# thygate/stable-diffusion-webui-depthmap-script

Hardware: NVIDIA H100
Metric: images/sec (higher is better)
Workload: dtype fp16

## Files before the change

### stable-diffusion-webui-depthmap-script_b200/csrc/attention_wgmma.cu

```cuda
#include <cuda.h>
#include <cuda_fp16.h>
#include <math.h>

#include "common.cuh"
#include "tc_common.cuh"

namespace dm {
using namespace tc;

__device__ __forceinline__ float ex2_approx(float x) {
    float y;
    asm("ex2.approx.ftz.f32 %0, %1;" : "=f"(y) : "f"(x));
    return y;
}

int make_tmap_2d(CUtensorMap *tm, const void *ptr, uint64_t rows, uint64_t cols, uint64_t ld, uint32_t box_rows, uint32_t box_cols);

struct AttnParams {
    int B, N, H;
    int C;
    float scale_log2e;
    const __half *bias;
    int bias_ld;
    __half *out;
    const float *rel_table;
    int nrd, gh, gw;
    int sub_stride;
};

constexpr int AT_BQ = 128, AT_BKV = 128, AT_D = 64, AT_STAGES = 2;
constexpr int AT_THREADS = 384;
constexpr int AT_Q_BYTES = AT_BQ * AT_D * 2;
constexpr int AT_KV_BYTES = AT_BKV * AT_D * 2;
constexpr int AT_K_OFF = AT_Q_BYTES;
constexpr int AT_V_OFF = AT_K_OFF + AT_STAGES * AT_KV_BYTES;
constexpr int AT_BAR_OFF = AT_V_OFF + AT_STAGES * AT_KV_BYTES;
constexpr int AT_TAB_OFF = AT_BAR_OFF + 64;
constexpr int AT_SMEM_MAX = 227 * 1024;
constexpr int AT_STAGERS = 96;

static inline int relpos_sub_stride(int gh, int gw) {
    const int span = gh < (AT_BQ - 1) / gw + 2 ? gh : (AT_BQ - 1) / gw + 2;
    return ((2 * span - 1) * (2 * gw - 1) + 1 + 3) & ~3;
}

template <int BIAS_MODE>
__global__ void __launch_bounds__(AT_THREADS, 1) attention_wgmma_kernel(const __grid_constant__ CUtensorMap tmQKV, AttnParams p) {
    extern __shared__ __align__(1024) uint8_t smem_raw[];
    uint8_t *sQ = smem_raw, *sK = smem_raw + AT_K_OFF, *sV = smem_raw + AT_V_OFF;
    uint64_t *bars = reinterpret_cast<uint64_t *>(smem_raw + AT_BAR_OFF);
    uint64_t *q_full = bars, *kv_full = bars + 1, *kv_empty = bars + 1 + AT_STAGES;
    float *s_tab = reinterpret_cast<float *>(smem_raw + AT_TAB_OFF);
    int *s_koff = reinterpret_cast<int *>(s_tab + AT_STAGES * p.sub_stride);

    const int warp = threadIdx.x >> 5, lane = threadIdx.x & 31;
    const int q0 = blockIdx.x * AT_BQ, h = blockIdx.y, b = blockIdx.z;
    const int num_kv = (p.N + AT_BKV - 1) / AT_BKV;
    const int row_base = b * p.N;

    if (threadIdx.x == 0) {
        prefetch_tmap(&tmQKV);
        mbar_init(q_full, 1);
        for (int s = 0; s < AT_STAGES; ++s) {
            mbar_init(&kv_full[s], BIAS_MODE == 2 ? 1 + AT_STAGERS : 1);
            mbar_init(&kv_empty[s], 8);
        }
        fence_barrier_init();
    }
    __syncthreads();

    if (warp < 4) {
        if (threadIdx.x == 0) {
            mbar_arrive_expect_tx(q_full, AT_Q_BYTES);
            tma_load_2d(sQ, &tmQKV, q_full, h * AT_D, row_base + q0);
            for (int j = 0; j < num_kv; ++j) {
                const int s = j % AT_STAGES;
                mbar_wait(&kv_empty[s], ((j / AT_STAGES) & 1) ^ 1);
                mbar_arrive_expect_tx(&kv_full[s], 2 * AT_KV_BYTES);
                tma_load_2d(sK + s * AT_KV_BYTES, &tmQKV, &kv_full[s], p.C + h * AT_D, row_base + j * AT_BKV);
                tma_load_2d(sV + s * AT_KV_BYTES, &tmQKV, &kv_full[s], 2 * p.C + h * AT_D, row_base + j * AT_BKV);
            }
        } else if (BIAS_MODE == 2 && warp >= 1) {
            const int st = threadIdx.x - 32, rw = 2 * p.gw - 1;
            const float *tab = p.rel_table + (size_t)h * p.nrd;
            const int qy_min = (max(q0, 1) - 1) / p.gw, qy_max = (min(q0 + AT_BQ, p.N) - 2) / p.gw;
            for (int j = 0; j < num_kv; ++j) {
                const int s = j % AT_STAGES, kbase = j * AT_BKV;
                const int k_lo = max(kbase, 1), k_hi = min(kbase + AT_BKV, p.N) - 1;
                const int ky_min = (k_lo - 1) / p.gw, ky_max = (k_hi - 1) / p.gw;
                const int lo = (qy_min - ky_max + p.gh - 1) * rw;
                const int cnt = (qy_max - qy_min + ky_max - ky_min + 1) * rw;
                float *sub = s_tab + s * p.sub_stride;
                int *kof = s_koff + s * AT_BKV;
                mbar_wait(&kv_empty[s], ((j / AT_STAGES) & 1) ^ 1);
                for (int i = st; i < cnt; i += AT_STAGERS) sub[i] = __ldg(tab + lo + i);
                if (st == 0) sub[p.sub_stride - 1] = __ldg(tab + p.nrd - 3);
                for (int k = st; k < AT_BKV; k += AT_STAGERS) {
                    const int t = min(max(kbase + k, k_lo), k_hi) - 1;
                    kof[k] = (t / p.gw) * rw + (t % p.gw) + lo;
                }
                mbar_arrive(&kv_full[s]);
            }
        }
        return;
    }

    const int wg = (warp >> 2) - 1, t = lane & 3;
    constexpr float LOG2E = 1.4426950408889634f;
    int qi[2];
    bool q_ok[2];
    const __half *brow[2] = {nullptr, nullptr};
    int rp_base[2] = {0, 0}, rp_mult[2] = {1, 1};
    float rp_k0[2] = {0.f, 0.f};
#pragma unroll
    for (int r = 0; r < 2; ++r) {
        qi[r] = q0 + wg * 64 + (warp & 3) * 16 + (lane >> 2) + 8 * r;
        q_ok[r] = qi[r] < p.N;
        const int qq = q_ok[r] ? qi[r] : 0;
        if (BIAS_MODE == 1) brow[r] = p.bias + ((size_t)h * p.N + qq) * p.bias_ld;
        if (BIAS_MODE == 2) {
            const float *tab = p.rel_table + (size_t)h * p.nrd;
            if (qq == 0) { rp_base[r] = p.sub_stride - 1; rp_mult[r] = 0; rp_k0[r] = __ldg(tab + p.nrd - 1); }
            else {
                const int tt = qq - 1, qy = tt / p.gw, qx = tt % p.gw;
                rp_base[r] = (qy + p.gh - 1) * (2 * p.gw - 1) + (qx + p.gw - 1);
                rp_k0[r] = __ldg(tab + p.nrd - 2);
            }
        }
    }
    float o[32];
#pragma unroll
    for (int i = 0; i < 32; ++i) o[i] = 0.f;
    float m_run[2] = {-INFINITY, -INFINITY}, l_run[2] = {0.f, 0.f};
    const uint64_t qdesc = make_desc_kmajor_sw128(smem_u32(sQ) + wg * (64 * 128));

    mbar_wait(q_full, 0);
    for (int j = 0; j < num_kv; ++j) {
        const int s = j % AT_STAGES;
        const int kbase = j * AT_BKV;
        mbar_wait(&kv_full[s], (j / AT_STAGES) & 1);
        float sc[64];
        const float *sub = s_tab + s * p.sub_stride;
        const int *kof = s_koff + s * AT_BKV;
        const uint64_t kdesc = make_desc_kmajor_sw128(smem_u32(sK + s * AT_KV_BYTES));
        wgmma_fence();
#pragma unroll
        for (int k = 0; k < AT_D / 16; ++k) wgmma_ss<AT_BKV>(sc, qdesc + (uint64_t)(2 * k), kdesc + (uint64_t)(2 * k), k != 0);
        wgmma_commit();
        wgmma_wait<0>();
        float mx[2] = {-INFINITY, -INFINITY};
#pragma unroll
        for (int c = 0; c < AT_BKV / 8; ++c) {
            const int k0 = kbase + 8 * c + 2 * t;
#pragma unroll
            for (int r = 0; r < 2; ++r) {
                float b0 = 0.f, b1 = 0.f;
                if (BIAS_MODE == 1) {
                    const float2 bf = __half22float2(__ldg(reinterpret_cast<const __half2 *>(brow[r] + k0)));
                    b0 = bf.x * LOG2E; b1 = bf.y * LOG2E;
                } else if (BIAS_MODE == 2) {
                    const int2 kk = *reinterpret_cast<const int2 *>(kof + 8 * c + 2 * t);
                    b0 = k0 == 0 ? rp_k0[r] : sub[rp_base[r] - rp_mult[r] * kk.x];
                    b1 = sub[rp_base[r] - rp_mult[r] * kk.y];
                }
                float u0 = fmaf(sc[4 * c + 2 * r], p.scale_log2e, b0), u1 = fmaf(sc[4 * c + 2 * r + 1], p.scale_log2e, b1);
                u0 = k0 < p.N ? u0 : -INFINITY;
                u1 = k0 + 1 < p.N ? u1 : -INFINITY;
                sc[4 * c + 2 * r] = u0; sc[4 * c + 2 * r + 1] = u1;
                mx[r] = fmaxf(mx[r], fmaxf(u0, u1));
            }
        }
        float alpha[2];
#pragma unroll
        for (int r = 0; r < 2; ++r) {
            mx[r] = fmaxf(mx[r], __shfl_xor_sync(0xffffffffu, mx[r], 1));
            mx[r] = fmaxf(mx[r], __shfl_xor_sync(0xffffffffu, mx[r], 2));
            const float m_new = fmaxf(m_run[r], mx[r]);
            alpha[r] = ex2_approx(m_run[r] - m_new);
            m_run[r] = m_new;
        }
        uint32_t pa[AT_BKV / 16][4];
        float ls[2] = {0.f, 0.f};
#pragma unroll
        for (int c = 0; c < AT_BKV / 8; ++c) {
#pragma unroll
            for (int r = 0; r < 2; ++r) {
                const float e0 = ex2_approx(sc[4 * c + 2 * r] - m_run[r]), e1 = ex2_approx(sc[4 * c + 2 * r + 1] - m_run[r]);
                const __half2 h2 = __floats2half2_rn(e0, e1);
                const float2 pr = __half22float2(h2);
                ls[r] += pr.x + pr.y;
                pa[c >> 1][(c & 1) * 2 + r] = *reinterpret_cast<const uint32_t *>(&h2);
            }
        }
#pragma unroll
        for (int r = 0; r < 2; ++r) l_run[r] = fmaf(l_run[r], alpha[r], ls[r]);
#pragma unroll
        for (int c = 0; c < AT_D / 8; ++c) { o[4 * c] *= alpha[0]; o[4 * c + 1] *= alpha[0]; o[4 * c + 2] *= alpha[1]; o[4 * c + 3] *= alpha[1]; }
        const uint32_t sv = smem_u32(sV + s * AT_KV_BYTES);
        wgmma_fence();
#pragma unroll
        for (int k = 0; k < AT_BKV / 16; ++k) wgmma_rs_n64_bt(o, pa[k], make_desc_mnmajor_sw128(sv + k * 16 * 128));
        wgmma_commit();
        wgmma_wait<0>();
        if (lane == 0) mbar_arrive(&kv_empty[s]);
    }
#pragma unroll
    for (int r = 0; r < 2; ++r) {
        float l = l_run[r];
        l += __shfl_xor_sync(0xffffffffu, l, 1);
        l += __shfl_xor_sync(0xffffffffu, l, 2);
        if (!q_ok[r]) continue;
        const float inv = 1.0f / l;
        __half *dst = p.out + (size_t)(row_base + qi[r]) * p.C + h * AT_D + 2 * t;
#pragma unroll
        for (int c = 0; c < AT_D / 8; ++c)
            *reinterpret_cast<__half2 *>(dst + 8 * c) = __floats2half2_rn(o[4 * c + 2 * r] * inv, o[4 * c + 2 * r + 1] * inv);
    }
}

template <int MODE>
static int launch_attn(const CUtensorMap &tm, const AttnParams &p, cudaStream_t stream) {
    const size_t tab = MODE == 2 ? (size_t)AT_STAGES * ((size_t)p.sub_stride * 4 + AT_BKV * 4) : 0;
    if (AT_TAB_OFF + tab > (size_t)AT_SMEM_MAX) { set_error("attention: relative-position window %d x %d too wide for the table sub-windows", p.gh, p.gw); return DM_E_UNSUPPORTED; }
    static PerDeviceFlag configured;
    if (!configured.test_and_set())
        DM_CUDA_CHECK(cudaFuncSetAttribute(attention_wgmma_kernel<MODE>, cudaFuncAttributeMaxDynamicSharedMemorySize, AT_SMEM_MAX));
    dim3 grid((p.N + AT_BQ - 1) / AT_BQ, p.H, p.B);
    attention_wgmma_kernel<MODE><<<grid, AT_THREADS, AT_TAB_OFF + tab, stream>>>(tm, p);
    DM_LAUNCH_CHECK("attention_wgmma_kernel");
    return DM_OK;
}

int attention_f16(const __half *qkv, AttnParams p, cudaStream_t stream, const float *rel_table = nullptr, int nrd = 0, int gh = 0, int gw = 0) {
    if (p.C != p.H * AT_D) { set_error("attention_f16: head_dim must be 64"); return DM_E_UNSUPPORTED; }
    CUtensorMap tm;
    int rc = make_tmap_2d(&tm, qkv, (uint64_t)p.B * p.N, (uint64_t)3 * p.C, (uint64_t)3 * p.C, AT_BQ, AT_D);
    if (rc) return rc;
    if (p.bias && (p.bias_ld % 8 != 0 || p.bias_ld < ((p.N + AT_BKV - 1) / AT_BKV) * AT_BKV)) {
        set_error("attention_f16: bias row pitch must be a multiple of 8 and cover whole 128-key tiles (got %d)", p.bias_ld);
        return DM_E_INVALID;
    }
    p.rel_table = rel_table; p.nrd = nrd; p.gh = gh; p.gw = gw; p.sub_stride = 0;
    if (rel_table) {
        if (gh < 1 || gw < 1 || (long long)gh * gw + 1 != p.N || (long long)nrd != (long long)(2 * gh - 1) * (2 * gw - 1) + 3) {
            set_error("attention_f16: relative-position mode needs N = gh*gw+1 and nrd = (2gh-1)(2gw-1)+3");
            return DM_E_INVALID;
        }
        p.sub_stride = relpos_sub_stride(gh, gw);
        return launch_attn<2>(tm, p, stream);
    }
    return p.bias ? launch_attn<1>(tm, p, stream) : launch_attn<0>(tm, p, stream);
}

constexpr int AS_K_OFF = 2 * AT_Q_BYTES;
constexpr int AS_V_OFF = AS_K_OFF + AT_STAGES * 2 * AT_KV_BYTES;
constexpr int AS_BAR_OFF = AS_V_OFF + AT_STAGES * 2 * AT_KV_BYTES;
constexpr int AS_SMEM = AS_BAR_OFF + 64;

__global__ void __launch_bounds__(AT_THREADS, 1) attention_split_kernel(const __grid_constant__ CUtensorMap tmQKV, AttnParams p) {
    extern __shared__ __align__(1024) uint8_t smem_raw[];
    uint8_t *sQ = smem_raw, *sK = smem_raw + AS_K_OFF, *sV = smem_raw + AS_V_OFF;
    uint64_t *bars = reinterpret_cast<uint64_t *>(smem_raw + AS_BAR_OFF);
    uint64_t *q_full = bars, *kv_full = bars + 1, *kv_empty = bars + 1 + AT_STAGES;

    const int warp = threadIdx.x >> 5, lane = threadIdx.x & 31;
    const int q0 = blockIdx.x * AT_BQ, h = blockIdx.y, b = blockIdx.z;
    const int num_kv = (p.N + AT_BKV - 1) / AT_BKV;
    const int row_base = b * p.N;
    const int lo = 3 * p.C;

    if (threadIdx.x == 0) {
        prefetch_tmap(&tmQKV);
        mbar_init(q_full, 1);
        for (int s = 0; s < AT_STAGES; ++s) { mbar_init(&kv_full[s], 1); mbar_init(&kv_empty[s], 8); }
        fence_barrier_init();
    }
    __syncthreads();

    if (warp < 4) {
        if (threadIdx.x == 0) {
            mbar_arrive_expect_tx(q_full, 2 * AT_Q_BYTES);
            tma_load_2d(sQ, &tmQKV, q_full, h * AT_D, row_base + q0);
            tma_load_2d(sQ + AT_Q_BYTES, &tmQKV, q_full, lo + h * AT_D, row_base + q0);
            for (int j = 0; j < num_kv; ++j) {
                const int s = j % AT_STAGES, r = row_base + j * AT_BKV;
                uint8_t *k = sK + s * 2 * AT_KV_BYTES, *v = sV + s * 2 * AT_KV_BYTES;
                mbar_wait(&kv_empty[s], ((j / AT_STAGES) & 1) ^ 1);
                mbar_arrive_expect_tx(&kv_full[s], 4 * AT_KV_BYTES);
                tma_load_2d(k, &tmQKV, &kv_full[s], p.C + h * AT_D, r);
                tma_load_2d(k + AT_KV_BYTES, &tmQKV, &kv_full[s], lo + p.C + h * AT_D, r);
                tma_load_2d(v, &tmQKV, &kv_full[s], 2 * p.C + h * AT_D, r);
                tma_load_2d(v + AT_KV_BYTES, &tmQKV, &kv_full[s], lo + 2 * p.C + h * AT_D, r);
            }
        }
        return;
    }

    const int wg = (warp >> 2) - 1, t = lane & 3;
    int qi[2];
#pragma unroll
    for (int r = 0; r < 2; ++r) qi[r] = q0 + wg * 64 + (warp & 3) * 16 + (lane >> 2) + 8 * r;
    float o[32];
#pragma unroll
    for (int i = 0; i < 32; ++i) o[i] = 0.f;
    float m_run[2] = {-INFINITY, -INFINITY}, l_run[2] = {0.f, 0.f};
    const uint64_t qh_desc = make_desc_kmajor_sw128(smem_u32(sQ) + wg * (64 * 128));
    const uint64_t ql_desc = make_desc_kmajor_sw128(smem_u32(sQ + AT_Q_BYTES) + wg * (64 * 128));

    mbar_wait(q_full, 0);
    for (int j = 0; j < num_kv; ++j) {
        const int s = j % AT_STAGES;
        const int kbase = j * AT_BKV;
        mbar_wait(&kv_full[s], (j / AT_STAGES) & 1);
        float sc[64];
        const uint32_t sk = smem_u32(sK + s * 2 * AT_KV_BYTES);
        const uint64_t kh_desc = make_desc_kmajor_sw128(sk), kl_desc = make_desc_kmajor_sw128(sk + AT_KV_BYTES);
        wgmma_fence();
#pragma unroll
        for (int k = 0; k < AT_D / 16; ++k) wgmma_ss<AT_BKV>(sc, ql_desc + (uint64_t)(2 * k), kh_desc + (uint64_t)(2 * k), k != 0);
#pragma unroll
        for (int k = 0; k < AT_D / 16; ++k) wgmma_ss<AT_BKV>(sc, qh_desc + (uint64_t)(2 * k), kl_desc + (uint64_t)(2 * k), 1);
#pragma unroll
        for (int k = 0; k < AT_D / 16; ++k) wgmma_ss<AT_BKV>(sc, qh_desc + (uint64_t)(2 * k), kh_desc + (uint64_t)(2 * k), 1);
        wgmma_commit();
        wgmma_wait<0>();
        float mx[2] = {-INFINITY, -INFINITY};
#pragma unroll
        for (int c = 0; c < AT_BKV / 8; ++c) {
            const int k0 = kbase + 8 * c + 2 * t;
#pragma unroll
            for (int r = 0; r < 2; ++r) {
                float u0 = sc[4 * c + 2 * r] * p.scale_log2e, u1 = sc[4 * c + 2 * r + 1] * p.scale_log2e;
                u0 = k0 < p.N ? u0 : -INFINITY;
                u1 = k0 + 1 < p.N ? u1 : -INFINITY;
                sc[4 * c + 2 * r] = u0; sc[4 * c + 2 * r + 1] = u1;
                mx[r] = fmaxf(mx[r], fmaxf(u0, u1));
            }
        }
        float alpha[2];
#pragma unroll
        for (int r = 0; r < 2; ++r) {
            mx[r] = fmaxf(mx[r], __shfl_xor_sync(0xffffffffu, mx[r], 1));
            mx[r] = fmaxf(mx[r], __shfl_xor_sync(0xffffffffu, mx[r], 2));
            const float m_new = fmaxf(m_run[r], mx[r]);
            alpha[r] = ex2_approx(m_run[r] - m_new);
            m_run[r] = m_new;
        }
        uint32_t ph[AT_BKV / 16][4], pl[AT_BKV / 16][4];
        float ls[2] = {0.f, 0.f};
#pragma unroll
        for (int c = 0; c < AT_BKV / 8; ++c) {
#pragma unroll
            for (int r = 0; r < 2; ++r) {
                const float e0 = ex2_approx(sc[4 * c + 2 * r] - m_run[r]) * 4096.f, e1 = ex2_approx(sc[4 * c + 2 * r + 1] - m_run[r]) * 4096.f;
                ls[r] += e0 + e1;
                const __half2 hi = __floats2half2_rn(e0, e1);
                const float2 hf = __half22float2(hi);
                const __half2 lo2 = __floats2half2_rn(e0 - hf.x, e1 - hf.y);
                ph[c >> 1][(c & 1) * 2 + r] = *reinterpret_cast<const uint32_t *>(&hi);
                pl[c >> 1][(c & 1) * 2 + r] = *reinterpret_cast<const uint32_t *>(&lo2);
            }
        }
#pragma unroll
        for (int r = 0; r < 2; ++r) l_run[r] = fmaf(l_run[r], alpha[r], ls[r]);
        float pv[32];
#pragma unroll
        for (int i = 0; i < 32; ++i) pv[i] = 0.f;
        const uint32_t sv = smem_u32(sV + s * 2 * AT_KV_BYTES);
        wgmma_fence();
#pragma unroll
        for (int k = 0; k < AT_BKV / 16; ++k) wgmma_rs_n64_bt(pv, pl[k], make_desc_mnmajor_sw128(sv + k * 16 * 128));
#pragma unroll
        for (int k = 0; k < AT_BKV / 16; ++k) wgmma_rs_n64_bt(pv, ph[k], make_desc_mnmajor_sw128(sv + AT_KV_BYTES + k * 16 * 128));
#pragma unroll
        for (int k = 0; k < AT_BKV / 16; ++k) wgmma_rs_n64_bt(pv, ph[k], make_desc_mnmajor_sw128(sv + k * 16 * 128));
        wgmma_commit();
        wgmma_wait<0>();
        if (lane == 0) mbar_arrive(&kv_empty[s]);
#pragma unroll
        for (int c = 0; c < AT_D / 8; ++c) {
            o[4 * c] = fmaf(o[4 * c], alpha[0], pv[4 * c]); o[4 * c + 1] = fmaf(o[4 * c + 1], alpha[0], pv[4 * c + 1]);
            o[4 * c + 2] = fmaf(o[4 * c + 2], alpha[1], pv[4 * c + 2]); o[4 * c + 3] = fmaf(o[4 * c + 3], alpha[1], pv[4 * c + 3]);
        }
    }
#pragma unroll
    for (int r = 0; r < 2; ++r) {
        float l = l_run[r];
        l += __shfl_xor_sync(0xffffffffu, l, 1);
        l += __shfl_xor_sync(0xffffffffu, l, 2);
        if (qi[r] >= p.N) continue;
        __half *dst = p.out + (size_t)(row_base + qi[r]) * (3 * p.C) + h * AT_D + 2 * t;
#pragma unroll
        for (int c = 0; c < AT_D / 8; ++c) {
            const float v0 = o[4 * c + 2 * r] / l, v1 = o[4 * c + 2 * r + 1] / l;
            const __half2 hi = __floats2half2_rn(v0, v1);
            const float2 hf = __half22float2(hi);
            *reinterpret_cast<__half2 *>(dst + 8 * c) = hi;
            *reinterpret_cast<__half2 *>(dst + p.C + 8 * c) = __floats2half2_rn(v0 - hf.x, v1 - hf.y);
            *reinterpret_cast<__half2 *>(dst + 2 * p.C + 8 * c) = hi;
        }
    }
}

int attention_split(const __half *qkv, AttnParams p, cudaStream_t stream) {
    if (p.C != p.H * AT_D || p.H < 1) { set_error("dm_attention_split: head_dim must be 64"); return DM_E_UNSUPPORTED; }
    if (p.N < 2 || p.B < 1 || !qkv || !p.out) { set_error("dm_attention_split: bad arguments (N >= 2 tokens, B >= 1)"); return DM_E_INVALID; }
    CUtensorMap tm;
    int rc = make_tmap_2d(&tm, qkv, (uint64_t)p.B * p.N, (uint64_t)9 * p.C, (uint64_t)9 * p.C, AT_BQ, AT_D);
    if (rc) return rc;
    static PerDeviceFlag configured;
    if (!configured.test_and_set())
        DM_CUDA_CHECK(cudaFuncSetAttribute(attention_split_kernel, cudaFuncAttributeMaxDynamicSharedMemorySize, AS_SMEM));
    dim3 grid((p.N + AT_BQ - 1) / AT_BQ, p.H, p.B);
    attention_split_kernel<<<grid, AT_THREADS, AS_SMEM, stream>>>(tm, p);
    DM_LAUNCH_CHECK("attention_split_kernel");
    return DM_OK;
}

}

extern "C" __attribute__((visibility("default"))) int dm_attention_split(const void *qkv, int B, int N, int H, float scale, void *out, void *stream) {
    dm::AttnParams p;
    memset(&p, 0, sizeof(p));
    p.B = B; p.N = N; p.H = H; p.C = H * 64;
    p.scale_log2e = scale * 1.4426950408889634f;
    p.out = (__half *)out;
    return dm::attention_split((const __half *)qkv, p, (cudaStream_t)stream);
}

extern "C" __attribute__((visibility("default"))) int dm_attention_f16(const void *qkv, int B, int N, int H, float scale, const void *bias, int bias_ld,
                                                                    void *out, void *stream) {
    dm::AttnParams p;
    p.B = B; p.N = N; p.H = H; p.C = H * 64;
    p.scale_log2e = scale * 1.4426950408889634f;
    p.bias = (const __half *)bias; p.bias_ld = bias_ld;
    p.out = (__half *)out;
    return dm::attention_f16((const __half *)qkv, p, (cudaStream_t)stream);
}

extern "C" __attribute__((visibility("default"))) int dm_attention_relpos_f16(const void *qkv, int B, int gh, int gw, int H, float scale,
                                                                           const float *rel_table_log2e, int nrd,
                                                                           void *out, void *stream) {
    dm::AttnParams p;
    p.B = B; p.N = gh * gw + 1; p.H = H; p.C = H * 64;
    p.scale_log2e = scale * 1.4426950408889634f;
    p.bias = nullptr; p.bias_ld = 0;
    p.out = (__half *)out;
    if (!rel_table_log2e) { dm::set_error("dm_attention_relpos_f16: table is NULL"); return DM_E_INVALID; }
    return dm::attention_f16((const __half *)qkv, p, (cudaStream_t)stream, rel_table_log2e, nrd, gh, gw);
}
```

Baseline: 318.4.

## Pipeline attention with ping-pong warpgroups, 3-stage KV, and narrow last tile

Restructures the attention main loop so each warpgroup issues the QK^T GEMM for tile j together with the PV GEMM for tile j-1. Named barriers make the two consumer warpgroups alternate, so one group's softmax overlaps the other's tensor-core work. It also deepens the K/V ring to three stages and moves registers from producer to consumer warps via setmaxnreg. It skips the idle second warpgroup on short final query blocks, and uses a narrow N=32 GEMM when the last key tile is small and a bias is present. Relative-position bias lookups use raw shared-memory addressing, and key-bound masking now applies only on the last tile. The cost is much more complex synchronisation, higher register pressure, and extra shared memory for the third stage, which could fail the table-size check on wide windows.

```diff
diff --git a/stable-diffusion-webui-depthmap-script_b200/csrc/attention_wgmma.cu b/stable-diffusion-webui-depthmap-script_b200/csrc/attention_wgmma.cu
--- a/stable-diffusion-webui-depthmap-script_b200/csrc/attention_wgmma.cu
+++ b/stable-diffusion-webui-depthmap-script_b200/csrc/attention_wgmma.cu
@@ -1,6 +1,8 @@
 #include <cuda.h>
 #include <cuda_fp16.h>
 #include <math.h>
+
+#include <type_traits>
 
 #include "common.cuh"
 #include "tc_common.cuh"
@@ -12,6 +14,12 @@
     float y;
     asm("ex2.approx.ftz.f32 %0, %1;" : "=f"(y) : "f"(x));
     return y;
+}
+
+__device__ __forceinline__ float lds_f32(uint32_t addr) {
+    float v;
+    asm volatile("ld.shared.f32 %0, [%1];" : "=f"(v) : "r"(addr));
+    return v;
 }
 
 int make_tmap_2d(CUtensorMap *tm, const void *ptr, uint64_t rows, uint64_t cols, uint64_t ld, uint32_t box_rows, uint32_t box_cols);
@@ -28,16 +36,19 @@
     int sub_stride;
 };
 
-constexpr int AT_BQ = 128, AT_BKV = 128, AT_D = 64, AT_STAGES = 2;
+constexpr int AT_BQ = 128, AT_BKV = 128, AT_D = 64;
+constexpr int AT_STAGES = 2;
+constexpr int AT_KV_STAGES = 3;
 constexpr int AT_THREADS = 384;
 constexpr int AT_Q_BYTES = AT_BQ * AT_D * 2;
 constexpr int AT_KV_BYTES = AT_BKV * AT_D * 2;
 constexpr int AT_K_OFF = AT_Q_BYTES;
-constexpr int AT_V_OFF = AT_K_OFF + AT_STAGES * AT_KV_BYTES;
-constexpr int AT_BAR_OFF = AT_V_OFF + AT_STAGES * AT_KV_BYTES;
-constexpr int AT_TAB_OFF = AT_BAR_OFF + 64;
+constexpr int AT_V_OFF = AT_K_OFF + AT_KV_STAGES * AT_KV_BYTES;
+constexpr int AT_BAR_OFF = AT_V_OFF + AT_KV_STAGES * AT_KV_BYTES;
+constexpr int AT_TAB_OFF = AT_BAR_OFF + 8 * (1 + 2 * AT_KV_STAGES + 1);
 constexpr int AT_SMEM_MAX = 227 * 1024;
 constexpr int AT_STAGERS = 96;
+constexpr int AT_NARROW = 32;
 
 static inline int relpos_sub_stride(int gh, int gw) {
     const int span = gh < (AT_BQ - 1) / gw + 2 ? gh : (AT_BQ - 1) / gw + 2;
@@ -49,33 +60,35 @@
     extern __shared__ __align__(1024) uint8_t smem_raw[];
     uint8_t *sQ = smem_raw, *sK = smem_raw + AT_K_OFF, *sV = smem_raw + AT_V_OFF;
     uint64_t *bars = reinterpret_cast<uint64_t *>(smem_raw + AT_BAR_OFF);
-    uint64_t *q_full = bars, *kv_full = bars + 1, *kv_empty = bars + 1 + AT_STAGES;
+    uint64_t *q_full = bars, *kv_full = bars + 1, *kv_empty = bars + 1 + AT_KV_STAGES;
     float *s_tab = reinterpret_cast<float *>(smem_raw + AT_TAB_OFF);
-    int *s_koff = reinterpret_cast<int *>(s_tab + AT_STAGES * p.sub_stride);
+    int *s_koff = reinterpret_cast<int *>(s_tab + AT_KV_STAGES * p.sub_stride);
 
     const int warp = threadIdx.x >> 5, lane = threadIdx.x & 31;
     const int q0 = blockIdx.x * AT_BQ, h = blockIdx.y, b = blockIdx.z;
     const int num_kv = (p.N + AT_BKV - 1) / AT_BKV;
     const int row_base = b * p.N;
+    const int n_wg = q0 + 64 < p.N ? 2 : 1;
 
     if (threadIdx.x == 0) {
         prefetch_tmap(&tmQKV);
         mbar_init(q_full, 1);
-        for (int s = 0; s < AT_STAGES; ++s) {
+        for (int s = 0; s < AT_KV_STAGES; ++s) {
             mbar_init(&kv_full[s], BIAS_MODE == 2 ? 1 + AT_STAGERS : 1);
-            mbar_init(&kv_empty[s], 8);
+            mbar_init(&kv_empty[s], 4 * n_wg);
         }
         fence_barrier_init();
     }
     __syncthreads();
 
     if (warp < 4) {
+        setmaxnreg_dec<40>();
         if (threadIdx.x == 0) {
             mbar_arrive_expect_tx(q_full, AT_Q_BYTES);
             tma_load_2d(sQ, &tmQKV, q_full, h * AT_D, row_base + q0);
             for (int j = 0; j < num_kv; ++j) {
-                const int s = j % AT_STAGES;
-                mbar_wait(&kv_empty[s], ((j / AT_STAGES) & 1) ^ 1);
+                const int s = j % AT_KV_STAGES;
+                mbar_wait(&kv_empty[s], ((j / AT_KV_STAGES) & 1) ^ 1);
                 mbar_arrive_expect_tx(&kv_full[s], 2 * AT_KV_BYTES);
                 tma_load_2d(sK + s * AT_KV_BYTES, &tmQKV, &kv_full[s], p.C + h * AT_D, row_base + j * AT_BKV);
                 tma_load_2d(sV + s * AT_KV_BYTES, &tmQKV, &kv_full[s], 2 * p.C + h * AT_D, row_base + j * AT_BKV);
@@ -85,14 +98,14 @@
             const float *tab = p.rel_table + (size_t)h * p.nrd;
             const int qy_min = (max(q0, 1) - 1) / p.gw, qy_max = (min(q0 + AT_BQ, p.N) - 2) / p.gw;
             for (int j = 0; j < num_kv; ++j) {
-                const int s = j % AT_STAGES, kbase = j * AT_BKV;
+                const int s = j % AT_KV_STAGES, kbase = j * AT_BKV;
                 const int k_lo = max(kbase, 1), k_hi = min(kbase + AT_BKV, p.N) - 1;
                 const int ky_min = (k_lo - 1) / p.gw, ky_max = (k_hi - 1) / p.gw;
                 const int lo = (qy_min - ky_max + p.gh - 1) * rw;
                 const int cnt = (qy_max - qy_min + ky_max - ky_min + 1) * rw;
                 float *sub = s_tab + s * p.sub_stride;
                 int *kof = s_koff + s * AT_BKV;
-                mbar_wait(&kv_empty[s], ((j / AT_STAGES) & 1) ^ 1);
+                mbar_wait(&kv_empty[s], ((j / AT_KV_STAGES) & 1) ^ 1);
                 for (int i = st; i < cnt; i += AT_STAGERS) sub[i] = __ldg(tab + lo + i);
                 if (st == 0) sub[p.sub_stride - 1] = __ldg(tab + p.nrd - 3);
                 for (int k = st; k < AT_BKV; k += AT_STAGERS) {
@@ -106,11 +119,13 @@
     }
 
     const int wg = (warp >> 2) - 1, t = lane & 3;
+    if (wg >= n_wg) return;
+    setmaxnreg_inc<232>();
     constexpr float LOG2E = 1.4426950408889634f;
     int qi[2];
     bool q_ok[2];
     const __half *brow[2] = {nullptr, nullptr};
-    int rp_base[2] = {0, 0}, rp_mult[2] = {1, 1};
+    int rp_base[2] = {0, 0}, rp_step[2] = {-4, -4};
     float rp_k0[2] = {0.f, 0.f};
 #pragma unroll
     for (int r = 0; r < 2; ++r) {
@@ -120,7 +135,7 @@
         if (BIAS_MODE == 1) brow[r] = p.bias + ((size_t)h * p.N + qq) * p.bias_ld;
         if (BIAS_MODE == 2) {
             const float *tab = p.rel_table + (size_t)h * p.nrd;
-            if (qq == 0) { rp_base[r] = p.sub_stride - 1; rp_mult[r] = 0; rp_k0[r] = __ldg(tab + p.nrd - 1); }
+            if (qq == 0) { rp_base[r] = p.sub_stride - 1; rp_step[r] = 0; rp_k0[r] = __ldg(tab + p.nrd - 1); }
             else {
                 const int tt = qq - 1, qy = tt / p.gw, qx = tt % p.gw;
                 rp_base[r] = (qy + p.gh - 1) * (2 * p.gw - 1) + (qx + p.gw - 1);
@@ -131,26 +146,41 @@
     float o[32];
 #pragma unroll
     for (int i = 0; i < 32; ++i) o[i] = 0.f;
-    float m_run[2] = {-INFINITY, -INFINITY}, l_run[2] = {0.f, 0.f};
+    float m_run[2] = {-INFINITY, -INFINITY}, l_run[2] = {0.f, 0.f}, alpha[2];
+    float sc[64];
+    uint32_t pa[AT_BKV / 16][4];
     const uint64_t qdesc = make_desc_kmajor_sw128(smem_u32(sQ) + wg * (64 * 128));
-
-    mbar_wait(q_full, 0);
-    for (int j = 0; j < num_kv; ++j) {
-        const int s = j % AT_STAGES;
-        const int kbase = j * AT_BKV;
-        mbar_wait(&kv_full[s], (j / AT_STAGES) & 1);
-        float sc[64];
-        const float *sub = s_tab + s * p.sub_stride;
+    const int last = num_kv - 1;
+    const bool narrow = BIAS_MODE != 0 && p.N - last * AT_BKV <= AT_NARROW;
+    const bool pingpong = n_wg == 2;
+
+    auto issue_s = [&](auto nc, int j) {
+        const uint64_t kdesc = make_desc_kmajor_sw128(smem_u32(sK + (j % AT_KV_STAGES) * AT_KV_BYTES));
+        if constexpr (decltype(nc)::value == AT_NARROW / 8) {
+            float (&s32)[16] = *reinterpret_cast<float (*)[16]>(sc);
+#pragma unroll
+            for (int k = 0; k < AT_D / 16; ++k) wgmma_ss<AT_NARROW>(s32, qdesc + (uint64_t)(2 * k), kdesc + (uint64_t)(2 * k), k != 0);
+        } else {
+#pragma unroll
+            for (int k = 0; k < AT_D / 16; ++k) wgmma_ss<AT_BKV>(sc, qdesc + (uint64_t)(2 * k), kdesc + (uint64_t)(2 * k), k != 0);
+        }
+        wgmma_commit();
+    };
+    auto issue_pv = [&](auto nc, int j) {
+        const uint32_t sv = smem_u32(sV + (j % AT_KV_STAGES) * AT_KV_BYTES);
+#pragma unroll
+        for (int k = 0; k < decltype(nc)::value / 2; ++k) wgmma_rs_n64_bt(o, pa[k], make_desc_mnmajor_sw128(sv + k * 16 * 128));
+        wgmma_commit();
+    };
+    auto softmax = [&](auto nc, auto last_tile, int j) {
+        constexpr int NC = decltype(nc)::value;
+        constexpr bool LAST = decltype(last_tile)::value;
+        const int s = j % AT_KV_STAGES, kbase = j * AT_BKV;
+        const uint32_t rowb[2] = {smem_u32(s_tab + s * p.sub_stride + rp_base[0]), smem_u32(s_tab + s * p.sub_stride + rp_base[1])};
         const int *kof = s_koff + s * AT_BKV;
-        const uint64_t kdesc = make_desc_kmajor_sw128(smem_u32(sK + s * AT_KV_BYTES));
-        wgmma_fence();
-#pragma unroll
-        for (int k = 0; k < AT_D / 16; ++k) wgmma_ss<AT_BKV>(sc, qdesc + (uint64_t)(2 * k), kdesc + (uint64_t)(2 * k), k != 0);
-        wgmma_commit();
-        wgmma_wait<0>();
         float mx[2] = {-INFINITY, -INFINITY};
 #pragma unroll
-        for (int c = 0; c < AT_BKV / 8; ++c) {
+        for (int c = 0; c < NC; ++c) {
             const int k0 = kbase + 8 * c + 2 * t;
 #pragma unroll
             for (int r = 0; r < 2; ++r) {
@@ -160,17 +190,18 @@
                     b0 = bf.x * LOG2E; b1 = bf.y * LOG2E;
                 } else if (BIAS_MODE == 2) {
                     const int2 kk = *reinterpret_cast<const int2 *>(kof + 8 * c + 2 * t);
-                    b0 = k0 == 0 ? rp_k0[r] : sub[rp_base[r] - rp_mult[r] * kk.x];
-                    b1 = sub[rp_base[r] - rp_mult[r] * kk.y];
+                    b0 = c == 0 && k0 == 0 ? rp_k0[r] : lds_f32(rowb[r] + kk.x * rp_step[r]);
+                    b1 = lds_f32(rowb[r] + kk.y * rp_step[r]);
                 }
                 float u0 = fmaf(sc[4 * c + 2 * r], p.scale_log2e, b0), u1 = fmaf(sc[4 * c + 2 * r + 1], p.scale_log2e, b1);
-                u0 = k0 < p.N ? u0 : -INFINITY;
-                u1 = k0 + 1 < p.N ? u1 : -INFINITY;
+                if (LAST) {
+                    u0 = k0 < p.N ? u0 : -INFINITY;
+                    u1 = k0 + 1 < p.N ? u1 : -INFINITY;
+                }
                 sc[4 * c + 2 * r] = u0; sc[4 * c + 2 * r + 1] = u1;
                 mx[r] = fmaxf(mx[r], fmaxf(u0, u1));
             }
         }
-        float alpha[2];
 #pragma unroll
         for (int r = 0; r < 2; ++r) {
             mx[r] = fmaxf(mx[r], __shfl_xor_sync(0xffffffffu, mx[r], 1));
@@ -179,10 +210,9 @@
             alpha[r] = ex2_approx(m_run[r] - m_new);
             m_run[r] = m_new;
         }
-        uint32_t pa[AT_BKV / 16][4];
         float ls[2] = {0.f, 0.f};
 #pragma unroll
-        for (int c = 0; c < AT_BKV / 8; ++c) {
+        for (int c = 0; c < NC; ++c) {
 #pragma unroll
             for (int r = 0; r < 2; ++r) {
                 const float e0 = ex2_approx(sc[4 * c + 2 * r] - m_run[r]), e1 = ex2_approx(sc[4 * c + 2 * r + 1] - m_run[r]);
@@ -194,16 +224,60 @@
         }
 #pragma unroll
         for (int r = 0; r < 2; ++r) l_run[r] = fmaf(l_run[r], alpha[r], ls[r]);
+    };
+    auto fence_operands = [&]() {
+#pragma unroll
+        for (int i = 0; i < 32; ++i) { asm volatile("" : "+f"(o[i])::"memory"); }
+#pragma unroll
+        for (int i = 0; i < 64; ++i) { asm volatile("" : "+f"(sc[i])::"memory"); }
+    };
+    auto rescale_o = [&]() {
 #pragma unroll
         for (int c = 0; c < AT_D / 8; ++c) { o[4 * c] *= alpha[0]; o[4 * c + 1] *= alpha[0]; o[4 * c + 2] *= alpha[1]; o[4 * c + 3] *= alpha[1]; }
-        const uint32_t sv = smem_u32(sV + s * AT_KV_BYTES);
+    };
+    auto turn_begin = [&](bool first) { if (pingpong && !(first && wg == 0)) named_bar_sync(1 + wg, 256); };
+    auto turn_end = [&](bool final_turn) { if (pingpong && !(final_turn && wg == 1)) named_bar_arrive(2 - wg, 256); };
+    auto step = [&](auto nc, auto last_tile, auto with_pv, int j) {
+        constexpr bool PV = decltype(with_pv)::value;
+        if constexpr (PV) rescale_o();
+        turn_begin(!PV);
         wgmma_fence();
-#pragma unroll
-        for (int k = 0; k < AT_BKV / 16; ++k) wgmma_rs_n64_bt(o, pa[k], make_desc_mnmajor_sw128(sv + k * 16 * 128));
-        wgmma_commit();
+        issue_s(nc, j);
+        if constexpr (PV) issue_pv(std::integral_constant<int, AT_BKV / 8>(), j - 1);
+        turn_end(false);
         wgmma_wait<0>();
-        if (lane == 0) mbar_arrive(&kv_empty[s]);
-    }
+        fence_operands();
+        if constexpr (PV) { if (lane == 0) mbar_arrive(&kv_empty[(j - 1) % AT_KV_STAGES]); }
+        softmax(nc, last_tile, j);
+    };
+    auto finish = [&](auto nc) {
+        rescale_o();
+        turn_begin(false);
+        wgmma_fence();
+        issue_pv(nc, last);
+        turn_end(true);
+        wgmma_wait<0>();
+        fence_operands();
+        if (lane == 0) mbar_arrive(&kv_empty[last % AT_KV_STAGES]);
+    };
+    using Wide = std::integral_constant<int, AT_BKV / 8>;
+    using Narrow = std::integral_constant<int, AT_NARROW / 8>;
+
+    mbar_wait(q_full, 0);
+    mbar_wait(&kv_full[0], 0);
+    using Last = std::true_type;
+    using Inner = std::false_type;
+    if (last > 0) step(Wide(), Inner(), std::false_type(), 0);
+    else if (narrow) step(Narrow(), Last(), std::false_type(), 0);
+    else step(Wide(), Last(), std::false_type(), 0);
+    for (int j = 1; j <= last; ++j) {
+        mbar_wait(&kv_full[j % AT_KV_STAGES], (j / AT_KV_STAGES) & 1);
+        if (j < last) step(Wide(), Inner(), std::true_type(), j);
+        else if (narrow) step(Narrow(), Last(), std::true_type(), j);
+        else step(Wide(), Last(), std::true_type(), j);
+    }
+    if (narrow) finish(Narrow());
+    else finish(Wide());
 #pragma unroll
     for (int r = 0; r < 2; ++r) {
         float l = l_run[r];
@@ -220,7 +294,7 @@
 
 template <int MODE>
 static int launch_attn(const CUtensorMap &tm, const AttnParams &p, cudaStream_t stream) {
-    const size_t tab = MODE == 2 ? (size_t)AT_STAGES * ((size_t)p.sub_stride * 4 + AT_BKV * 4) : 0;
+    const size_t tab = MODE == 2 ? (size_t)AT_KV_STAGES * ((size_t)p.sub_stride * 4 + AT_BKV * 4) : 0;
     if (AT_TAB_OFF + tab > (size_t)AT_SMEM_MAX) { set_error("attention: relative-position window %d x %d too wide for the table sub-windows", p.gh, p.gw); return DM_E_UNSUPPORTED; }
     static PerDeviceFlag configured;
     if (!configured.test_and_set())
```

New measurement: 325.3 (median of 6 runs). 2.2% higher.
